# BioinfoMachineLearning/bio-diffusion

Hardware: NVIDIA B200
Metric: molecules/sec (1000-step sample) (higher is better)
Workload: dtype bf16x2 (split hi+lo operands, f32 accumulate; <=1e-4 of the fp32 reference)

## Files before the change

### bio-diffusion_b200/bdiff/_lib.py

```python
from __future__ import annotations

import ctypes as C
import os

_HERE = os.path.dirname(os.path.abspath(__file__))
LIB_PATH = os.path.join(_HERE, "libbdiff_sm100.so")

MODE_PARITY_FP32 = 0
MODE_TENSOR = 1


class BdiffError(RuntimeError):
    pass


class Config(C.Structure):
    _fields_ = [("num_h", C.c_int32), ("num_context", C.c_int32), ("num_layers", C.c_int32),
                ("h_hidden", C.c_int32), ("chi_hidden", C.c_int32), ("e_hidden", C.c_int32),
                ("xi_hidden", C.c_int32), ("mode", C.c_int32)]


PROTOTYPES = {
    "bdiff_abi_version": (C.c_int32, []),
    "bdiff_create": (C.c_int32, [C.POINTER(Config), C.POINTER(C.c_void_p)]),
    "bdiff_destroy": (None, [C.c_void_p]),
    "bdiff_last_error": (C.c_char_p, [C.c_void_p]),
    "bdiff_set_weight": (C.c_int32, [C.c_void_p, C.c_void_p, C.c_char_p, C.c_void_p, C.POINTER(C.c_int64), C.c_int32]),
    "bdiff_weights_missing": (C.c_int32, [C.c_void_p]),
    "bdiff_prepare": (C.c_int32, [C.c_void_p, C.c_void_p]),
    "bdiff_selftest_split": (C.c_int32, [C.c_void_p, C.c_int32, C.c_void_p, C.c_void_p, C.c_void_p]),
    "bdiff_selftest_pair": (C.c_int32, [C.c_void_p, C.c_void_p, C.c_void_p, C.c_void_p]),
    "bdiff_plan_topology": (C.c_int32, [C.c_void_p, C.c_void_p, C.c_int32, C.c_int64, C.c_void_p, C.c_void_p,
                                        C.POINTER(C.c_int64)]),
    "bdiff_edge_index": (C.c_int32, [C.c_void_p, C.c_void_p, C.c_void_p]),
    "bdiff_denoise_forward": (C.c_int32, [C.c_void_p, C.c_void_p, C.c_void_p, C.c_void_p, C.c_void_p, C.c_void_p]),
    "bdiff_profile_forward": (C.c_int32, [C.c_void_p, C.c_void_p, C.c_void_p, C.c_void_p, C.c_void_p, C.c_void_p,
                                          C.POINTER(C.c_float)]),
    "bdiff_debug_tap": (C.c_int32, [C.c_void_p, C.c_void_p, C.c_char_p, C.c_void_p, C.POINTER(C.c_int64),
                                    C.POINTER(C.c_int64)]),
    "bdiff_reverse_step": (C.c_int32, [C.c_void_p, C.c_void_p, C.c_void_p, C.c_void_p, C.c_void_p, C.c_void_p,
                                       C.c_void_p, C.c_void_p]),
    "bdiff_decode_z0": (C.c_int32, [C.c_void_p, C.c_void_p, C.c_void_p, C.c_void_p, C.c_void_p, C.c_void_p,
                                    C.c_void_p, C.c_void_p]),
    "bdiff_center_noise": (C.c_int32, [C.c_void_p, C.c_void_p, C.c_void_p, C.c_void_p, C.c_void_p]),
    "bdiff_check": (C.c_int32, [C.c_void_p, C.c_void_p]),
    "bdiff_check_stability": (C.c_int32, [C.c_void_p] * 4 + [C.c_int32, C.c_int32] + [C.c_void_p] * 3 + [C.c_float] * 3 +
                              [C.c_void_p, C.c_int32, C.c_void_p, C.c_void_p, C.c_void_p]),
    "bdiff_bond_orders": (C.c_int32, [C.c_void_p] * 5 + [C.c_int32, C.c_int32] + [C.c_void_p] * 3 + [C.c_float] * 3 +
                          [C.c_int32, C.c_void_p]),
    "bdiff_collate_count": (C.c_int32, [C.c_void_p, C.c_void_p, C.c_void_p, C.c_int32, C.c_int32, C.c_void_p]),
    "bdiff_collate_packed": (C.c_int32, [C.c_void_p] * 6 + [C.c_int32, C.c_int32, C.c_int32] + [C.c_void_p] * 4),
    "bdiff_prepare_context": (C.c_int32, [C.c_void_p] * 6 + [C.c_int64, C.c_int64, C.c_int32, C.c_void_p]),
    "bdiff_optimizer_chunk": (C.c_int32, []),
    "bdiff_optimizer_step": (C.c_int32, [C.c_void_p, C.c_void_p, C.c_void_p, C.c_void_p, C.c_int32, C.c_void_p, C.c_void_p,
                                         C.c_void_p]),
    "bdiff_param_floats": (C.c_int64, [C.c_void_p]),
    "bdiff_param_layout": (C.c_int32, [C.c_void_p, C.c_char_p, C.POINTER(C.c_int64), C.POINTER(C.c_int64)]),
    "bdiff_train_precision": (C.c_int32, [C.c_void_p, C.c_int32]),
    "bdiff_train_variant": (C.c_int32, [C.c_void_p, C.c_int32]),
    "bdiff_train_timing": (C.c_int32, [C.c_void_p, C.c_void_p, C.c_int32, C.c_char_p, C.c_int64]),
    "bdiff_train_forward": (C.c_int32, [C.c_void_p] * 7),
    "bdiff_train_backward": (C.c_int32, [C.c_void_p] * 4),
    "bdiff_nan_guard_count": (C.c_int32, [C.c_void_p, C.c_void_p, C.POINTER(C.c_int64), C.c_int32]),
    "bdiff_launch_count": (C.c_int64, [C.c_void_p]),
# ... 33 lines not shown
```

### bio-diffusion_b200/csrc/bdiff_api.cu

```cuda
#include <algorithm>
#include <cstdarg>
#include <cstdio>
#include <cstdlib>
#include <cstring>
#include <map>
#include <string>
#include <utility>
#include <vector>

#include "../../include/bdiff.h"
#include "bdiff_handle.h"

using namespace bdiff;

namespace {

thread_local std::string g_create_error;


}

namespace {

void gcp_names(std::map<std::string, bool>& seen, const std::string& p, bool ff, bool vout) {
// ... 139 lines not shown
               o_fbar = take(Np * 12), o_h = take(Np * 256), o_chi = take(Np * 96), o_PI = take(Np * kPStride),
               o_PJ = take(Np * kPStride), o_agg = take(Np * kMsg), o_hp = take(Np * 32),
               o_e = take(Ep * d.Ed), o_xie = take(Ep * d.Xd * 3), o_fr = take(Ep * 9), o_pjt = take(Np * 256),
               o_mid = take(h->cfg.mode == BDIFF_MODE_TENSOR ? (Ep / 128) * kMsg : 0),
               o_flag = take(64);
  cudaError_t e = h->work_buf.ensure(off * sizeof(float));
  if (e != cudaSuccess) return e;
  float* b = static_cast<float*>(h->work_buf.p);
  Work& w = h->work;
  w.x_init = b + o_xi; w.x = b + o_x; w.h_in = b + o_hin; w.chi_in = b + o_chin; w.fbar = b + o_fbar;
  w.h = b + o_h; w.chi = b + o_chi; w.PI = b + o_PI; w.PJ = b + o_PJ; w.agg = b + o_agg; w.hproj = b + o_hp;
  w.e = b + o_e; w.xi = b + o_xie; w.frames = b + o_fr;
  w.PJT = h->cfg.mode == BDIFF_MODE_TENSOR ? b + o_pjt : nullptr;
  w.mid = h->cfg.mode == BDIFF_MODE_TENSOR ? b + o_mid : nullptr;
  w.npad = (int)Np;
  w.nan_flag = reinterpret_cast<int*>(b + o_flag);
  w.dbg = nullptr;
  if (getenv("BDIFF_TIMING")) {
    e = h->dbg_buf.ensure(2 * 256 * 64 * sizeof(long long));
    if (e != cudaSuccess) return e;
    w.dbg = static_cast<long long*>(h->dbg_buf.p);
  }
  e = h->eps_buf.ensure(Np * (3 + d.F) * sizeof(float));
  if (e != cudaSuccess) return e;
  return h->tu_buf.ensure(256);
}

}

extern "C" {

int32_t bdiff_abi_version(void) { return BDIFF_ABI_VERSION; }

const char* bdiff_last_error(const bdiff_handle* h) { return h ? h->err.c_str() : g_create_error.c_str(); }

int32_t bdiff_create(const bdiff_config* cfg, bdiff_handle** out) {
  if (!cfg || !out) { g_create_error = "null argument"; return BDIFF_EINVAL; }
  *out = nullptr;
  if (cfg->h_hidden != 256 || cfg->chi_hidden != 32) { g_create_error = "h_hidden must be 256 and chi_hidden 32"; return BDIFF_EINVAL; }
  if (cfg->e_hidden < 4 || cfg->e_hidden > 64 || cfg->e_hidden % 4) { g_create_error = "e_hidden must be a multiple of 4 in [4,64]"; return BDIFF_EINVAL; }
  if (cfg->xi_hidden < 4 || cfg->xi_hidden > 16 || cfg->xi_hidden % 4) { g_create_error = "xi_hidden must be a multiple of 4 in [4,16]"; return BDIFF_EINVAL; }
  if (cfg->num_h < 1 || cfg->num_context < 0 || cfg->num_h + 1 + cfg->num_context > 28) { g_create_error = "num_h + 1 + num_context must be in [2,28]"; return BDIFF_EINVAL; }
  if (cfg->num_layers < 1 || cfg->num_layers > 64) { g_create_error = "num_layers out of range"; return BDIFF_EINVAL; }
  if (cfg->mode != BDIFF_MODE_PARITY_FP32 && cfg->mode != BDIFF_MODE_TENSOR) { g_create_error = "unknown mode"; return BDIFF_EINVAL; }
  int dev_count = 0;
  if (cudaGetDeviceCount(&dev_count) != cudaSuccess || dev_count == 0) {
    g_create_error = "no CUDA device: libbdiff_sm100 has no CPU fallback";
    return BDIFF_ECUDA;
  }
  cudaDeviceProp prop{};
  int dev = 0;
  cudaGetDevice(&dev);
  cudaGetDeviceProperties(&prop, dev);
  if (prop.major != 10) {
    g_create_error = "libbdiff_sm100 is built for sm_100a (B200) only; found compute capability " +
                     std::to_string(prop.major) + "." + std::to_string(prop.minor);
    return BDIFF_ECUDA;
  }
  bdiff_handle* h = new bdiff_handle();
  h->cfg = *cfg;
  Dims& d = h->d;
  d.F = cfg->num_h; d.C = cfg->num_context; d.Hin = d.F + 1 + d.C; d.Ed = cfg->e_hidden; d.Xd = cfg->xi_hidden;
  d.hid0 = (64 + d.Xd) / 4;
  d.K0 = round_up(d.Ed + d.hid0 + 9, 4);
  d.Ke = round_up(1 + d.Xd + 9, 4);
  d.Kn = round_up(d.Hin + 32 + 9, 4);
// ... 563 lines not shown
```

### bio-diffusion_b200/csrc/bdiff_edge_tc.cuh

```cuda
#pragma once
#include "bdiff_kernels.h"
#include "bdiff_slab.cuh"

namespace bdiff {

constexpr int TMT = 128;
constexpr int TC_SLOT = 2 * 160 * 32;
constexpr int TC_NSLOT = 5;
constexpr int TM_S = 0, TM_U0 = 256, TM_U1 = 288, TM_MV = 320, TM_VD0 = 416;
constexpr int TM_EX = 416, TM_EX_STRIDE = 40;

__host__ __device__ inline int tc_k0_steps(int Ed, int Xd) {
  return (Ed + (64 + Xd) / 4 + 9 + 15) / 16;
}
__host__ __device__ inline size_t tc_edge_stream_bytes(int Ed, int Xd) {
  return (size_t)tc_k0_steps(Ed, Xd) * 2 * 256 * 32 + 3 * ((size_t)16 * 2 * 320 * 32 + 2 * 2 * 256 * 32) + (size_t)16 * 2 * 32 * 32;
}

struct TcBars {
  uint64_t full[TC_NSLOT], empty[TC_NSLOT], pfull[TC_NSLOT], a_ready, d_full, wbar, u_free;
  uint64_t item_full[2], item_empty[2], peer_empty[2], tile_done;
  alignas(16) int item[2][4];
  uint32_t tmem_ptr;
  uint32_t pad_;
};

constexpr int TC_EPI = 256;

struct alignas(16) SmallW {
  float Wd0x[16 * 20];
  float Wf0x[16 * 3];
  float Wu0[20 * 32];
  float Wdk[3][32 * 8];
  float Wfk[3][32 * 3];
  float Wuk[3][8 * 32];
  float bg[4][32];
  float bk[3][256];
  float wa[256];
  float ba[4];
};

struct EdgeTail : TcBars {
  float2 wbuf[2][8][2][32];
  SmallW sw;
  float sAttn[2][TMT];
  int sRow[TMT], sCol[TMT], sB[TMT], sNa[TMT];
  uint32_t winfo[8];
};

template <int HP, bool FIRST, bool LAST>
__device__ __forceinline__ void gate_update(uint32_t tl, int half, int ucol, const float* __restrict__ vdp,
                                            const float* __restrict__ Wu, const float* __restrict__ bgp,
                                            const float* __restrict__ Wdn, const float* __restrict__ Wfn,
// ... 101 lines not shown
```

### bio-diffusion_b200/csrc/bdiff_kernels.h

```cpp
#pragma once
#include <cuda_runtime.h>
#include <stddef.h>

#include "bdiff_common.cuh"

namespace bdiff {

struct Work {
  float* x_init;
  float* x;
  float* h_in;
  float* chi_in;
  float* fbar;
  float* h;
  float* chi;
  float* PI;
  float* PJ;
  float* PJT;
  int npad;
  float* agg;
  float* mid;
  float* hproj;
  float* e;
  float* xi;
  float* frames;
  int* nan_flag;
  long long* dbg;
};

cudaError_t configure_kernels();
size_t edge_smem_bytes();
size_t node_smem_bytes();

void launch_prep(cudaStream_t st, const Plan& p, const Dims& d, const float* xh, const float* t_nodes,
                 const float* coef_table, const int* step_ptr, const float* ctx, const Work& w);
void launch_edge_embed(cudaStream_t st, const Plan& p, const Dims& d, const EmbedW& ew, const Work& w);
void launch_node_embed(cudaStream_t st, const Plan& p, const Dims& d, const EmbedW& ew, const LayerW& l0,
                       const Work& w);
void launch_edge_message(cudaStream_t st, const Plan& p, const Dims& d, const LayerW& lw, const Work& w);
void launch_node_update(cudaStream_t st, const Plan& p, const Dims& d, const LayerW& lw, const LayerW& wn,
                        const EmbedW& ew, const Work& w, int last);
void launch_finalize(cudaStream_t st, const Plan& p, const Dims& d, const Work& w, float* out);
void launch_step(cudaStream_t st, const Plan& p, const Dims& d, int mode, const float* z, const float* eps,
                 const float* noise_x, const float* noise_h, const float* coef_table, const int* step_ptr,
                 float* out);
void launch_edge_index(cudaStream_t st, const Plan& p, long long* out);
void launch_edge_rc(cudaStream_t st, const Plan& p, int4* out, long long n);
struct PackJob {
  float* dst;
  const float* src;
  int dst_ld, src_ld, col0, ncols, kpad, nout;
  int block0;
};
void launch_pack_multi(cudaStream_t st, const PackJob* jobs_dev, int njobs, int total_blocks);

bool tc_supported(int Ed, int Xd);
size_t tc_blob_bytes(int Ed, int Xd);
size_t tc_node_blob_bytes();
void launch_tc_pack(cudaStream_t st, const LayerW& lw, const Dims& d, unsigned char* blob);
void launch_tc_pack_node(cudaStream_t st, const LayerW& lw, const LayerW& wn, const EmbedW& ew, const Dims& d, int last,
                         unsigned char* blob);
struct LayerSched {
  const LayerW* layers;
  const unsigned char* edge_blob;
  size_t edge_blob_stride;
  const unsigned char* node_blob;
  size_t node_blob_stride;
  int L, TE, TN;
  int nitems;
  int* sched;
  int* err;
  const int2* edge_dep;
  const int2* node_dep;
  const int* items;
};
cudaError_t tc_layers_configure();
void launch_layers_tc(cudaStream_t st, const Plan& p, const Dims& d, const EmbedW& ew, const LayerSched& q,
                      const Work& w, int num_sms);
cudaError_t selftest_configure();
cudaError_t selftest_pair_configure();
size_t selftest_pair_img_bytes();
void launch_umma_selftest_pair(cudaStream_t st, const float* A, const float* W, unsigned char* img_scratch, float* C);
size_t selftest_img_bytes();
void launch_umma_selftest_split(cudaStream_t st, const float* A, const float* W, unsigned char* img_scratch, float* C,
                                int variant);

}
```

### bio-diffusion_b200/csrc/bdiff_layers_tc.cu

```cuda
#include "bdiff_node_tc.cuh"

namespace bdiff {

__device__ __forceinline__ int ld_acquire_gpu(const int* p) {
  int v;
  asm volatile("ld.acquire.gpu.global.s32 %0, [%1];" : "=r"(v) : "l"(p) : "memory");
  return v;
}
__device__ __forceinline__ void st_release_gpu(int* p, int v) {
  asm volatile("st.release.gpu.global.s32 [%0], %1;" ::"l"(p), "r"(v) : "memory");
}

union LayersTail {
  TcBars bars;
  EdgeTail edge;
  NodeTail node;
};
constexpr size_t LAYERS_SMEM_BYTES = XE_BLOCKS * (size_t)X_BLOCK + TC_NSLOT * (size_t)TC_SLOT + sizeof(LayersTail) + 1024;
static_assert(LAYERS_SMEM_BYTES <= 232448, "shared memory budget of the layer megakernel");

constexpr int LAYERS_THREADS = 384;
constexpr int LAYERS_REG_COMPUTE = 200, LAYERS_REG_SERVICE = 96;
static_assert(256 * LAYERS_REG_COMPUTE + 128 * LAYERS_REG_SERVICE <= 168 * LAYERS_THREADS, "setmaxnreg pool");

// ... 16 lines not shown
}

template <int ED, int XD>
__global__ void __cluster_dims__(2, 1, 1) __launch_bounds__(LAYERS_THREADS, 1)
    k_layers_tc(Plan p, Dims d, EmbedW ew, LayerSched q, Work w) {
  constexpr int HID0 = (64 + XD) / 4;
  constexpr int H2 = HID0 / 2;
  constexpr int K0RAW = ED + HID0 + 9;
  constexpr int K0S = (K0RAW + 15) / 16;
  static_assert(HID0 % 2 == 0 && H2 * 3 <= 32 && HID0 + 9 <= 32 && ED % 16 == 0, "layout");

  extern __shared__ unsigned char smem_raw[];
  unsigned char* smem = smem_raw + ((1024u - (smem_u32(smem_raw) & 1023u)) & 1023u);
  unsigned char* X = smem;
  unsigned char* ring = smem + XE_BLOCKS * X_BLOCK;
  unsigned char* tail = ring + TC_NSLOT * TC_SLOT;
  TcBars& B = *reinterpret_cast<TcBars*>(tail);
  const int tid = threadIdx.x, warp = tid >> 5, lane = tid & 31;
  const int hid0 = d.hid0;
  const int per_layer = q.TE + q.TN;
  const int total_items = q.nitems;
  int* const flags = q.sched + 2;
  const uint32_t rank = cluster_ctarank();
  const bool leader = rank == 0;

  if (tid == 0) {
    for (int i = 0; i < TC_NSLOT; ++i) { mbar_init(&B.full[i], 1); mbar_init(&B.empty[i], 1); mbar_init(&B.pfull[i], 1); }
    for (int i = 0; i < 2; ++i) {
      mbar_init(&B.item_full[i], 1); mbar_init(&B.item_empty[i], leader ? TC_EPI + 1 : TC_EPI + 2); mbar_init(&B.peer_empty[i], 1);
    }
    mbar_init(&B.tile_done, TC_EPI);
    mbar_init(&B.a_ready, leader ? TC_EPI + 1 : TC_EPI);
    mbar_init(&B.d_full, 1);
    mbar_init(&B.wbar, 1);
    mbar_init(&B.u_free, leader ? TC_EPI + 1 : TC_EPI);
    mbar_fence_init();
  }
  cluster_sync_all();
  if (warp == 8) tmem_alloc2(&B.tmem_ptr, 512);
  tc_fence_before();
  __syncthreads();
  tc_fence_after();
  const uint32_t tmem = B.tmem_ptr;
  const uint32_t a_ready_leader = mapa_u32(&B.a_ready, 0), u_free_leader = mapa_u32(&B.u_free, 0);

  if (warp == 8) {
    asm volatile("setmaxnreg.dec.sync.aligned.u32 %0;\n" ::"n"(LAYERS_REG_SERVICE));
    if (lane == 0) {
      uint32_t ci = 0;
      for (uint32_t k = 0;; ++k) {
        const uint32_t slot = k & 1;
        mbar_wait_backoff(&B.item_empty[slot], ((k >> 1) & 1) ^ 1);
        int type = -1, layer = 0, tile = 0;
        if (leader) {
          mbar_wait_backoff(&B.peer_empty[slot], (k >> 1) & 1);
          const int qi = atomicAdd(q.sched, 1);
          int pair = 0;
          if (qi < total_items) {
            const int it = __ldg(q.items + qi);
            type = (it >> 30) & 1; layer = (it >> 24) & 63; pair = it & 0xffffff;
          }
          B.item[slot][0] = type; B.item[slot][1] = layer; B.item[slot][2] = 2 * pair;
          st_cluster_v4(mapa_u32(&B.item[slot][0], 1), type, layer, 2 * pair + 1, 0);
          mbar_arrive(&B.item_full[slot]);
          mbar_arrive_remote(mapa_u32(&B.item_full[slot], 1));
          tile = 2 * pair;
// ... 3 lines not shown
          type = B.item[slot][0]; layer = B.item[slot][1]; tile = B.item[slot][2];
        }
        (void)tile;
        if (type < 0) break;
        const unsigned char* blob = type == 0 ? q.edge_blob + (size_t)layer * q.edge_blob_stride + rank * (q.edge_blob_stride / 2)
                                              : q.node_blob + (size_t)layer * q.node_blob_stride + rank * (q.node_blob_stride / 2);
        size_t off = 0;
        auto push = [&](uint32_t bytes) {
          const uint32_t s = ci % TC_NSLOT;
          mbar_wait_backoff(&B.empty[s], ((ci / TC_NSLOT) & 1) ^ 1);
          mbar_expect_tx(&B.full[s], bytes);
          bulk_g2s(ring + s * TC_SLOT, blob + off, bytes, &B.full[s]);
          off += bytes;
          ++ci;
        };
        if (type == 0) {
#include "edge_tile_producer.inc"
        } else {
          const int last = layer == q.L - 1;
#include "node_r4_tile_producer.inc"
        }
      }
    }
  } else if (warp == 9 && !leader) {
    asm volatile("setmaxnreg.dec.sync.aligned.u32 %0;\n" ::"n"(LAYERS_REG_SERVICE));
    if (lane < TC_NSLOT) {
      const uint32_t pfull0 = mapa_u32(&B.pfull[0], 0);
      uint32_t ci = 0;
      for (uint32_t k = 0;; ++k) {
        const uint32_t slot = k & 1;
        mbar_wait_cluster(&B.item_full[slot], (k >> 1) & 1);
        const int type = B.item[slot][0], layer = B.item[slot][1], tile = B.item[slot][2];
        if (type < 0) break;
        const uint32_t nch = type == 0 ? K0S + 3 * 18 + 4 : (layer == q.L - 1 ? 73u : 100u);
        for (uint32_t cc = ci + ((lane + TC_NSLOT - ci % TC_NSLOT) % TC_NSLOT); cc < ci + nch; cc += TC_NSLOT) {
          mbar_wait_backoff(&B.full[lane], (cc / TC_NSLOT) & 1);
          mbar_arrive_remote_relaxed(pfull0 + lane * 8);
        }
        ci += nch;
        if (lane == 0) {
          mbar_wait_backoff(&B.tile_done, k & 1);
          __threadfence();
          if (tile < (type == 0 ? q.TE : q.TN))
            st_release_gpu(flags + (size_t)layer * per_layer + (type == 0 ? tile : q.TE + tile), 1);
          mbar_arrive(&B.item_empty[slot]);
        }
      }
    }
  } else if (warp == 9) {
    asm volatile("setmaxnreg.dec.sync.aligned.u32 %0;\n" ::"n"(LAYERS_REG_SERVICE));
    if (lane == 0) {
      TcBars& T = B;
      const uint32_t i256 = umma_idesc_bf16_m256(256), i64 = umma_idesc_bf16_m256(64), i32 = umma_idesc_bf16_m256(32);
      const uint32_t xaddr = smem_u32(X), raddr = smem_u32(ring);
      uint32_t ci = 0, pa = 0, pu = 0;
      long long wcyc = 0, acyc = 0;
      auto wait_a = [&]() {
        if (!leader) return;
        const long long t0 = w.dbg ? clock64() : 0;
        mbar_wait_backoff(&B.a_ready, pa); pa ^= 1;
        tc_fence_after();
        if (w.dbg) acyc += clock64() - t0;
      };
      auto wait_w = [&]() -> uint32_t {
        const uint32_t s = ci % TC_NSLOT, par = (ci / TC_NSLOT) & 1;
        const long long t0 = w.dbg ? clock64() : 0;
        mbar_wait_backoff(&B.full[s], par);
        mbar_wait_backoff(&B.pfull[s], par);
        if (w.dbg) wcyc += clock64() - t0;
        return raddr + s * TC_SLOT;
      };
      auto done_w = [&]() { if (leader) umma_commit_pair(&B.empty[ci % TC_NSLOT]); ++ci; };
      auto commit_d = [&]() { if (leader) umma_commit_pair(&B.d_full); };
      auto mma = [&](uint32_t dcol, uint64_t ad, uint64_t bd, uint32_t idesc, bool acc) { if (leader) umma_bf16_pair(tmem + dcol, ad, bd, idesc, acc); };
      auto ngemm = [&](int NL, uint32_t dcol, bool fresh, int umode) {
        for (int ks = 0; ks < 16; ++ks) {
          const uint32_t a = xaddr + (ks >> 2) * R5_BLOCK + (ks & 3) * 32;
          const uint64_t v0 = umma_desc_sw128(a), v1 = umma_desc_sw128(a + 4096);
          const uint32_t wb0 = wait_w();
          for (int pl = 0; pl < 2; ++pl) {
            const uint32_t wb = wb0 + pl * NL * 32;
            const bool first = ks == 0 && pl == 0;
            const uint64_t bs = umma_desc_k16(wb, NL * 16, 128);
            mma(dcol, v0, bs, i256, fresh ? !first : true);
            mma(dcol, v1, bs, i256, true);
            if (umode) {
              const uint64_t bu = umma_desc_k16(wb + 128 * 16, NL * 16, 128);
              mma(NM_U, v0, bu, i32, umode == 2 ? !first : true);
              mma(NM_U, v1, bu, i32, true);
            }
          }
          done_w();
        }
      };
      auto nextra = [&]() {
        for (int ks = 0; ks < 2; ++ks) {
          const uint32_t a = xaddr + 4 * R5_BLOCK + ks * 32;
          const uint64_t v0 = umma_desc_sw128(a), v1 = umma_desc_sw128(a + 4096);
          const uint32_t wb0 = wait_w();
          for (int pl = 0; pl < 2; ++pl) {
            const uint32_t wb = wb0 + pl * 128 * 32;
            mma(NM_S, v0, umma_desc_k16(wb, 128 * 16, 128), i256, true);
            mma(NM_S, v1, umma_desc_k16(wb, 128 * 16, 128), i256, true);
          }
          done_w();
        }
// ... 15 lines not shown
          long long* o = w.dbg + 256 * 64 + 148 * 64 + (size_t)blockIdx.x * 8 + (k - 2) * 4;
          o[0] = (type << 30) | (layer << 24) | tile; o[1] = clock64() - tstart; o[2] = wcyc; o[3] = acyc;
        }
        mbar_wait_backoff(&B.tile_done, k & 1);
        __threadfence();
        if (tile < (type == 0 ? q.TE : q.TN))
          st_release_gpu(flags + (size_t)layer * per_layer + (type == 0 ? tile : q.TE + tile), 1);
        mbar_arrive(&B.item_empty[slot]);
      }
    }
  } else if (warp == 10) {
    asm volatile("setmaxnreg.dec.sync.aligned.u32 %0;\n" ::"n"(LAYERS_REG_SERVICE));
    if (lane == 0 && !leader) {
      uint32_t pa = 0, pu = 0;
      for (uint32_t k = 0;; ++k) {
        const uint32_t slot = k & 1;
        mbar_wait_cluster(&B.item_full[slot], (k >> 1) & 1);
        const int type = B.item[slot][0], layer = B.item[slot][1];
        if (type < 0) break;
        const bool has_u = type == 1 && layer != q.L - 1;
        const int nph = type == 0 ? 8 : 6;
        for (int ph = 0; ph < nph; ++ph) {
          if (has_u && ph == 4) { mbar_wait_backoff(&B.u_free, pu); pu ^= 1; mbar_arrive_remote_relaxed(u_free_leader); }
          mbar_wait_backoff(&B.a_ready, pa); pa ^= 1;
          mbar_arrive_remote_relaxed(a_ready_leader);
        }
        mbar_arrive(&B.item_empty[slot]);
      }
    }
  } else if (warp >= 11) {
    asm volatile("setmaxnreg.dec.sync.aligned.u32 %0;\n" ::"n"(LAYERS_REG_SERVICE));
  } else {
    asm volatile("setmaxnreg.inc.sync.aligned.u32 %0;\n" ::"n"(LAYERS_REG_COMPUTE));
    uint32_t pd = 0, pw = 0;
    int cur_type = -1, cur_layer = -1;
    int es = 0;
    long long* stamp = nullptr;
    auto PH = [&]() { if (stamp && tid == 0 && es < 32) stamp[es] = clock64(); ++es; };
    auto wait_d = [&]() { PH(); mbar_wait(&B.d_full, pd); pd ^= 1; tc_fence_after(); PH(); };
    auto publish = [&]() { fence_proxy_async(); tc_fence_before(); mbar_arrive(&B.a_ready); PH(); };
    bool stamped[2] = {false, false};
    const uint32_t tl = tmem + ((uint32_t)((warp & 3) * 32) << 16);
    auto sz = [](int n) { return (uint32_t)((n * 4 + 15) & ~15); };
    for (uint32_t k = 0;; ++k) {
      const uint32_t slot = k & 1;
      mbar_wait_cluster(&B.item_full[slot], (k >> 1) & 1);
      const int type = B.item[slot][0], layer = B.item[slot][1], tile = B.item[slot][2];
      if (type < 0) break;
      const bool real = tile < (type == 0 ? q.TE : q.TN);
      if (tid == 0 && w.dbg && k < 16) {
        w.dbg[(size_t)blockIdx.x * 64 + 4 * k] = (type << 30) | (layer << 24) | tile;
        w.dbg[(size_t)blockIdx.x * 64 + 4 * k + 1] = clock64();
      }
      if (type != cur_type || layer != cur_layer) {
        named_bar_sync(3, TC_EPI);
        if (tid == 0) {
          const LayerW lw = q.layers[layer];
          if (type == 0) {
            SmallW& s = reinterpret_cast<EdgeTail*>(tail)->sw;
            mbar_expect_tx(&B.wbar, sz(XD * HID0) + sz(XD * 3) + sz(HID0 * 32) +
                                        3 * (sz(256) + sz(256) + sz(256) + sz(96) + sz(32)) + sz(32) + sz(256) + sz(1));
            auto cp = [&](float* dst, const float* src, int n) { bulk_g2s(dst, src, sz(n), &B.wbar); };
            cp(s.Wd0x, lw.Wd0x, XD * HID0); cp(s.Wf0x, lw.Wf0x, XD * 3); cp(s.Wu0, lw.Wu0, HID0 * 32);
            for (int kk = 0; kk < 3; ++kk) {
              cp(s.Wdk[kk], lw.Wdk[kk], 256); cp(s.Wuk[kk], lw.Wuk[kk], 256); cp(s.bk[kk], lw.bk[kk], 256);
              cp(s.Wfk[kk], lw.Wfk[kk], 96); cp(s.bg[kk + 1], lw.bgk[kk], 32);
            }
            cp(s.bg[0], lw.bg0, 32); cp(s.wa, lw.wa, 256); cp(s.ba, lw.ba, 1);
          } else {
            const int last = layer == q.L - 1;
            const LayerW wn = q.layers[last ? layer : layer + 1];
            SmallWR4& s = reinterpret_cast<NodeTail*>(tail)->sw;
// ... 93 lines not shown
```

### bio-diffusion_b200/csrc/bdiff_tc_pack.cu

```cuda
#include "bdiff_node_tc.cuh"

namespace bdiff {

size_t tc_blob_bytes(int Ed, int Xd) { return tc_edge_stream_bytes(Ed, Xd); }
size_t tc_node_blob_bytes() { return tc_node_stream_bytes(0); }

__global__ void k_pack_edge_slabs(LayerW lw, Dims d, unsigned char* __restrict__ blob, size_t half_bytes) {
  const int K0S = tc_k0_steps(d.Ed, d.Xd);
  const long long rows_g = 16 * 320 + 2 * 256;
  const long long total_rows = (long long)K0S * 256 + 3 * rows_g + 16 * 32;
  const long long idx = (long long)blockIdx.x * blockDim.x + threadIdx.x;
  if (idx >= total_rows * 16) return;
  long long row = idx >> 4;
  const int kk = (int)(idx & 15);
  size_t base = 0;
  int NL, n, k, cta, local;
  float v;
  if (row < (long long)K0S * 256) {
    const int step = (int)(row / 256);
    n = (int)(row % 256); NL = 128; cta = n >> 7; local = n & 127; base = (size_t)step * 2 * 128 * 32; k = step * 16 + kk;
    v = k < d.K0 ? lw.W0e[(size_t)k * 256 + n] : 0.f;
  } else {
    row -= (long long)K0S * 256;
    base = (size_t)K0S * 2 * 128 * 32;
    const size_t bytes_g = (size_t)16 * 2 * 160 * 32 + 2 * 2 * 128 * 32;
    if (row < 3 * rows_g) {
      const int gi = (int)(row / rows_g);
      long long rr = row - gi * rows_g;
      base += gi * bytes_g;
      if (rr < 16 * 320) {
        const int step = (int)(rr / 320);
        n = (int)(rr % 320); NL = 160; base += (size_t)step * 2 * 160 * 32; k = step * 16 + kk;
        const float* wprev = gi == 0 ? lw.Wg0 : lw.Wgk[gi - 1];
        const float* wthis = lw.Wgk[gi];
        const bool odd = ((gi + 1) & 1) != 0;
        if (n < 256) { v = lw.Wk[gi][(size_t)k * 256 + n]; cta = n >> 7; local = n & 127; }
        else if (n < 288) { v = odd ? wprev[(size_t)k * 32 + (n - 256)] : -wthis[(size_t)k * 32 + (n - 256)]; cta = 0; local = 128 + (n - 256); }
        else { v = odd ? -wthis[(size_t)k * 32 + (n - 288)] : wprev[(size_t)k * 32 + (n - 288)]; cta = 1; local = 128 + (n - 288); }
      } else {
        rr -= 16 * 320;
        const int step = (int)(rr / 256);
        n = (int)(rr % 256); NL = 128; cta = n >> 7; local = n & 127;
        base += (size_t)16 * 2 * 160 * 32 + (size_t)step * 2 * 128 * 32; k = 256 + step * 16 + kk;
        v = k < kKM ? lw.Wk[gi][(size_t)k * 256 + n] : 0.f;
      }
    } else {
      row -= 3 * rows_g;
      base += 3 * bytes_g;
      const int step = (int)(row / 32);
      n = (int)(row % 32); NL = 16; cta = n >> 4; local = n & 15; base += (size_t)step * 2 * 16 * 32; k = step * 16 + kk;
      v = lw.Wgk[2][(size_t)k * 32 + n];
    }
  }
  slab_store(blob + (size_t)cta * half_bytes + base, NL, local, kk, v);
}

__global__ void k_pack_node_slabs(LayerW lw, LayerW wn, EmbedW ew, Dims d, int last, unsigned char* __restrict__ blob,
                                  size_t half_bytes) {
  const long long idx = (long long)blockIdx.x * blockDim.x + threadIdx.x;
  long long row = idx >> 4;
  const int kk = (int)(idx & 15);
  size_t base = 0;
  int NL = 0, n = 0, k = 0, cta = 0, local = 0;
  float v = 0.f;
  bool found = false;
  auto seg = [&](int steps, int NN) -> bool {
    if (found) return false;
    const long long rows = (long long)steps * NN;
    const int nl = NN == 256 ? 128 : (NN == 288 ? 144 : 16);
    if (row < rows) {
      const int step = (int)(row / NN);
// ... 43 lines not shown
```

### bio-diffusion_b200/csrc/edge_tile_epilogue.inc

```
      const long long g = (long long)tile * TMT + r;
      constexpr int PV = HID0 * 3 + 9, PF4 = (PV + 3) / 4, PLD = PF4 * 4 + 1;
      constexpr int XF4 = XD * 3 / 4, XLD = XD * 3 + 1;
      static_assert(K0S <= 8 && TMT * XLD * 4 <= 2 * X_BLOCK && TMT * PLD * 4 <= 3 * X_BLOCK, "staging areas");
      float* sFx = reinterpret_cast<float*>(X + 2 * X_BLOCK);
      float* sFp = reinterpret_cast<float*>(X + 6 * X_BLOCK);
      const int4 rc = __ldg(p.edge_rc + g);
      float f[9];
      {
        constexpr int F4_ROW = ED / 4;
        const float4* eb = reinterpret_cast<const float4*>(w.e + (size_t)tile * TMT * ED);
        const float4* xb = reinterpret_cast<const float4*>(w.xi + (size_t)tile * TMT * XD * 3);
        float4 ev[TMT * F4_ROW / TC_EPI], xv[TMT * XF4 / TC_EPI];
#pragma unroll
        for (int i = 0; i < TMT * F4_ROW / TC_EPI; ++i) ev[i] = eb[i * TC_EPI + tid];
#pragma unroll
        for (int i = 0; i < TMT * XF4 / TC_EPI; ++i) xv[i] = xb[i * TC_EPI + tid];
#pragma unroll
        for (int qq = 0; qq < 9; ++qq) f[qq] = w.frames[(size_t)g * 9 + qq];
        if (half == 0) { T.sRow[r] = rc.x; T.sCol[r] = rc.y; T.sB[r] = rc.z; T.sNa[r] = rc.w; }
#pragma unroll
        for (int i = 0; i < TMT * F4_ROW / TC_EPI; ++i) {
          const int idx = i * TC_EPI + tid;
          const int rr = idx / F4_ROW, kk = (idx % F4_ROW) * 4;
          xe_store4(X, rr, kk, ev[i].x, ev[i].y, ev[i].z, ev[i].w);
// ... 98 lines not shown
        auto prefetch = [&](int c) {
          const float* pc = pjt + c * 1024;
#pragma unroll
          for (int i = 0; i < 32; ++i) pj[i] = pc[i * 32];
#pragma unroll
          for (int qq = 0; qq < 8; ++qq) pa[qq] = *reinterpret_cast<const float4*>(pi + half * 128 + c * 32 + qq * 4);
        };
        prefetch(0);
        wait_d();
        for (int c = 0; c < 4; ++c) {
          const int c0 = half * 128 + c * 32;
          float v[32];
          tmem_ld32(tl + TM_S + c0, v);
#pragma unroll
          for (int qq = 0; qq < 8; ++qq) {
            v[qq * 4 + 0] += pa[qq].x + pj[qq * 4 + 0]; v[qq * 4 + 1] += pa[qq].y + pj[qq * 4 + 1];
            v[qq * 4 + 2] += pa[qq].z + pj[qq * 4 + 2]; v[qq * 4 + 3] += pa[qq].w + pj[qq * 4 + 3];
          }
          if (c < 3) prefetch(c + 1);
#pragma unroll
          for (int qq = 0; qq < 16; ++qq) {
            const float2 p0 = silu_acc2(make_float2(v[2 * qq], v[2 * qq + 1]));
            v[2 * qq] = p0.x; v[2 * qq + 1] = p0.y;
          }
#pragma unroll
          for (int qq = 0; qq < 4; ++qq) xe_store8(X, r, c0 + qq * 8, v + qq * 8);
        }
      }
      publish();

      float vd[24], vdf[9];
      float2 adot2 = make_float2(0.f, 0.f);
      for (int k = 1; k <= 3; ++k) {
        wait_d();
        float part[33], other[33];
        if (k == 1) {
          float vd0[HID0 * 3];
          {
            float t0[64];
            float* t1 = t0 + 32;
            tmem_ld64(tl + TM_VD0, t0);
#pragma unroll
            for (int i = 0; i < H2 * 3; ++i) { vd0[i] = t0[i]; vd0[H2 * 3 + i] = t1[i]; }
          }
          tc_fence_before();
          named_bar_sync(3, TC_EPI);
          tc_fence_after();
          gate_update<HID0, true, false>(tl, half, TM_U0, vd0, sw.Wu0, sw.bg[0], sw.Wdk[0], sw.Wfk[0], part);
        } else {
          gate_update<8, false, false>(tl, half, ((k - 1) & 1) ? TM_U1 : TM_U0, vd, sw.Wuk[k - 2], sw.bg[k - 1],
                                       sw.Wdk[k - 1], sw.Wfk[k - 1], part);
        }
        pair_exchange33(tl, half, part, other);
#pragma unroll
        for (int i = 0; i < 24; ++i) vd[i] = half == 0 ? part[i] + other[i] : other[i] + part[i];
#pragma unroll
        for (int i = 0; i < 9; ++i) vdf[i] = half == 0 ? part[24 + i] + other[24 + i] : other[24 + i] + part[24 + i];
        {
          float a[16];
          if (half == 0) {
#pragma unroll
            for (int h = 0; h < 8; ++h) a[h] = safe_norm3(vd[h * 3], vd[h * 3 + 1], vd[h * 3 + 2]);
#pragma unroll
            for (int i = 0; i < 8; ++i) {
              const int ch = i / 3, ax = i - ch * 3;
              a[8 + i] = f[ax * 3] * vdf[ch * 3] + f[ax * 3 + 1] * vdf[ch * 3 + 1] + f[ax * 3 + 2] * vdf[ch * 3 + 2];
            }
// ... 166 lines not shown
```

### bio-diffusion_b200/csrc/edge_tile_mma.inc

```
        {
          const uint32_t xe = xaddr + XE_EXTRA * X_BLOCK;
          wait_a();
          for (int ks = 0; ks < K0S; ++ks) {
            const uint64_t ah = umma_desc_sw128(xaddr + (ks >> 2) * X_BLOCK + (ks & 3) * 32);
            const uint64_t al = umma_desc_sw128(xaddr + (XE_LO + (ks >> 2)) * X_BLOCK + (ks & 3) * 32);
            const uint32_t bh = wait_w(), bl = bh + 128 * 32;
            mma(TM_S, ah, umma_desc_k16(bh, 128 * 16, 128), i256, ks > 0);
            mma(TM_S, al, umma_desc_k16(bh, 128 * 16, 128), i256, true);
            mma(TM_S, ah, umma_desc_k16(bl, 128 * 16, 128), i256, true);
            done_w();
          }
          commit_d();
          for (int k = 1; k <= 3; ++k) {
            wait_a();
            for (int ks = 0; ks < 16; ++ks) {
              const uint64_t ah = umma_desc_sw128(xaddr + (ks >> 2) * X_BLOCK + (ks & 3) * 32);
              const uint64_t al = umma_desc_sw128(xaddr + (XE_LO + (ks >> 2)) * X_BLOCK + (ks & 3) * 32);
              const uint32_t bh = wait_w(), bl = bh + 160 * 32;
              mma(TM_S, ah, umma_desc_k16(bh, 160 * 16, 128), i256, ks > 0);
              mma(TM_U0, ah, umma_desc_k16(bh + 128 * 16, 160 * 16, 128), i64, k == 1 ? ks > 0 : true);
              mma(TM_S, al, umma_desc_k16(bh, 160 * 16, 128), i256, true);
              mma(TM_U0, al, umma_desc_k16(bh + 128 * 16, 160 * 16, 128), i64, true);
              mma(TM_S, ah, umma_desc_k16(bl, 160 * 16, 128), i256, true);
              mma(TM_U0, ah, umma_desc_k16(bl + 128 * 16, 160 * 16, 128), i64, true);
              done_w();
            }
            commit_d();
            wait_a();
            for (int ks = 0; ks < 2; ++ks) {
              const uint64_t ah = umma_desc_sw128(xe + ks * 32), al = umma_desc_sw128(xe + 64 + ks * 32);
              const uint32_t bh = wait_w(), bl = bh + 128 * 32;
              mma(TM_S, ah, umma_desc_k16(bh, 128 * 16, 128), i256, true);
              mma(TM_S, al, umma_desc_k16(bh, 128 * 16, 128), i256, true);
              mma(TM_S, ah, umma_desc_k16(bl, 128 * 16, 128), i256, true);
              done_w();
            }
            commit_d();
          }
          wait_a();
          for (int c = 0; c < 4; ++c) {
            const uint32_t wb = wait_w();
            for (int s4 = 0; s4 < 4; ++s4) {
              const int ks = c * 4 + s4;
              const uint64_t ah = umma_desc_sw128(xaddr + (ks >> 2) * X_BLOCK + (ks & 3) * 32);
              const uint64_t al = umma_desc_sw128(xaddr + (XE_LO + (ks >> 2)) * X_BLOCK + (ks & 3) * 32);
              const uint32_t bh = wb + s4 * 1024, bl = bh + 512;
              mma(TM_U1, ah, umma_desc_k16(bh, 16 * 16, 128), i32, true);
              mma(TM_U1, al, umma_desc_k16(bh, 16 * 16, 128), i32, true);
              mma(TM_U1, ah, umma_desc_k16(bl, 16 * 16, 128), i32, true);
            }
            done_w();
          }
          commit_d();
        }
```

### bio-diffusion_b200/csrc/edge_tile_producer.inc

```
        for (int ks = 0; ks < K0S; ++ks) push(2 * 128 * 32);
        for (int k = 0; k < 3; ++k) {
          for (int ks = 0; ks < 16; ++ks) push(2 * 160 * 32);
          for (int ks = 0; ks < 2; ++ks) push(2 * 128 * 32);
        }
        for (int c = 0; c < 4; ++c) push(4 * 2 * 16 * 32);
```

### include/bdiff.h

```cpp
#ifndef BDIFF_H_
#define BDIFF_H_

#include <stdint.h>

#ifdef __cplusplus
extern "C" {
#endif

#define BDIFF_OK 0
#define BDIFF_EINVAL (-1)
#define BDIFF_ECUDA (-2)
#define BDIFF_ESTATE (-3)
#define BDIFF_ENOMEM (-4)

#define BDIFF_ABI_VERSION 1

#if defined(__GNUC__)
#define BDIFF_API __attribute__((visibility("default")))
#else
#define BDIFF_API
#endif

#define BDIFF_MODE_PARITY_FP32 0
#define BDIFF_MODE_TENSOR 1

typedef struct bdiff_handle bdiff_handle;

typedef struct bdiff_config {
  int32_t num_h;
  int32_t num_context;
  int32_t num_layers;
  int32_t h_hidden;
  int32_t chi_hidden;
  int32_t e_hidden;
  int32_t xi_hidden;
  int32_t mode;
} bdiff_config;

BDIFF_API int32_t bdiff_abi_version(void);

BDIFF_API int32_t bdiff_create(const bdiff_config* cfg, bdiff_handle** out);
BDIFF_API void bdiff_destroy(bdiff_handle* h);
BDIFF_API const char* bdiff_last_error(const bdiff_handle* h);

BDIFF_API int32_t bdiff_set_weight(bdiff_handle* h, void* stream, const char* name, const float* data,
                         const int64_t* shape, int32_t ndim);
BDIFF_API int32_t bdiff_weights_missing(const bdiff_handle* h);

BDIFF_API int32_t bdiff_prepare(bdiff_handle* h, void* stream);

BDIFF_API int32_t bdiff_selftest_split(void* stream, int32_t variant, const float* A, const float* W, float* C);

BDIFF_API int32_t bdiff_selftest_pair(void* stream, const float* A, const float* W, float* C);

BDIFF_API int32_t bdiff_plan_topology(bdiff_handle* h, void* stream, int32_t num_mols, int64_t num_nodes,
                            const int64_t* batch_index, const uint8_t* mask, int64_t* num_edges_host);

BDIFF_API int32_t bdiff_edge_index(bdiff_handle* h, void* stream, int64_t* edge_index);

BDIFF_API int32_t bdiff_denoise_forward(bdiff_handle* h, void* stream, const float* xh, const float* t,
                              const float* context, float* net_out);

BDIFF_API int32_t bdiff_profile_forward(bdiff_handle* h, void* stream, const float* xh, const float* t,
                                        const float* context, float* net_out, float* ms_host);

BDIFF_API int32_t bdiff_debug_tap(bdiff_handle* h, void* stream, const char* which, float* dst, int64_t* rows,
                                  int64_t* cols);

BDIFF_API int32_t bdiff_reverse_step(bdiff_handle* h, void* stream, float* z, const float* context,
                                     const float* noise_x, const float* noise_h, const float* coef_table,
                                     const int32_t* step_index);

BDIFF_API int32_t bdiff_decode_z0(bdiff_handle* h, void* stream, const float* z0, const float* context,
                                  const float* noise_x, const float* noise_h, const float* coef, float* xh);

BDIFF_API int32_t bdiff_center_noise(bdiff_handle* h, void* stream, const float* noise_x, const float* noise_h,
                                     float* z);

BDIFF_API int32_t bdiff_check(bdiff_handle* h, void* stream);

#define BDIFF_OPT_MAX_QUEUE 120
#define BDIFF_OPT_STATE_WORDS (8 + BDIFF_OPT_MAX_QUEUE)
typedef struct bdiff_opt_tensor {
  float* param;
  const float* grad;
  float* exp_avg;
// ... 55 lines not shown
```

Before: 60.86.

## Split edge GCP weight stream so U-gate GEMM completes early on own barrier

Repacks the edge-tile weight stream so the 32-column U/gate weights for each GCP are streamed as separate chunks ahead of the 256-column scalar weights. The MMA warp computes the U accumulator first and signals a new u_full barrier, letting the epilogue start its vector work while the scalar GEMM is still running, instead of waiting on a single combined commit. This changes the packed blob layout, the chunk count and the producer sequence, and adds a host-visible layout query. It risks more pipeline chunks and smaller per-MMA N for the U part.

```diff
diff --git a/bio-diffusion_b200/bdiff/_lib.py b/bio-diffusion_b200/bdiff/_lib.py
--- a/bio-diffusion_b200/bdiff/_lib.py
+++ b/bio-diffusion_b200/bdiff/_lib.py
@@ -30,6 +30,7 @@
     "bdiff_prepare": (C.c_int32, [C.c_void_p, C.c_void_p]),
     "bdiff_selftest_split": (C.c_int32, [C.c_void_p, C.c_int32, C.c_void_p, C.c_void_p, C.c_void_p]),
     "bdiff_selftest_pair": (C.c_int32, [C.c_void_p, C.c_void_p, C.c_void_p, C.c_void_p]),
+    "bdiff_tc_edge_stream_layout": (C.c_int32, [C.c_int32, C.c_int32, C.POINTER(C.c_int64)]),
     "bdiff_plan_topology": (C.c_int32, [C.c_void_p, C.c_void_p, C.c_int32, C.c_int64, C.c_void_p, C.c_void_p,
                                         C.POINTER(C.c_int64)]),
     "bdiff_edge_index": (C.c_int32, [C.c_void_p, C.c_void_p, C.c_void_p]),
diff --git a/bio-diffusion_b200/csrc/bdiff_api.cu b/bio-diffusion_b200/csrc/bdiff_api.cu
--- a/bio-diffusion_b200/csrc/bdiff_api.cu
+++ b/bio-diffusion_b200/csrc/bdiff_api.cu
@@ -195,6 +195,12 @@
 
 int32_t bdiff_abi_version(void) { return BDIFF_ABI_VERSION; }
 
+int32_t bdiff_tc_edge_stream_layout(int32_t e_hidden, int32_t xi_hidden, int64_t* out) {
+  if (!out || !tc_supported(e_hidden, xi_hidden)) return BDIFF_EINVAL;
+  tc_edge_stream_layout(e_hidden, xi_hidden, out);
+  return 0;
+}
+
 const char* bdiff_last_error(const bdiff_handle* h) { return h ? h->err.c_str() : g_create_error.c_str(); }
 
 int32_t bdiff_create(const bdiff_config* cfg, bdiff_handle** out) {
diff --git a/bio-diffusion_b200/csrc/bdiff_edge_tc.cuh b/bio-diffusion_b200/csrc/bdiff_edge_tc.cuh
--- a/bio-diffusion_b200/csrc/bdiff_edge_tc.cuh
+++ b/bio-diffusion_b200/csrc/bdiff_edge_tc.cuh
@@ -10,15 +10,31 @@
 constexpr int TM_S = 0, TM_U0 = 256, TM_U1 = 288, TM_MV = 320, TM_VD0 = 416;
 constexpr int TM_EX = 416, TM_EX_STRIDE = 40;
 
-__host__ __device__ inline int tc_k0_steps(int Ed, int Xd) {
+__host__ __device__ constexpr int tc_k0_steps(int Ed, int Xd) {
   return (Ed + (64 + Xd) / 4 + 9 + 15) / 16;
 }
-__host__ __device__ inline size_t tc_edge_stream_bytes(int Ed, int Xd) {
+__host__ __device__ constexpr size_t tc_edge_stream_bytes(int Ed, int Xd) {
   return (size_t)tc_k0_steps(Ed, Xd) * 2 * 256 * 32 + 3 * ((size_t)16 * 2 * 320 * 32 + 2 * 2 * 256 * 32) + (size_t)16 * 2 * 32 * 32;
 }
 
+constexpr uint32_t TC_EC_S = 2 * 128 * 32, TC_EC_U = 4 * 2 * 32 * 32, TC_EC_G4 = 4 * 2 * 16 * 32;
+constexpr int TC_EC_PER_GCP = 4 + 16 + 2;
+__host__ __device__ constexpr int tc_edge_tile_chunks(int k0s) { return k0s + 3 * TC_EC_PER_GCP + 4; }
+__host__ __device__ constexpr uint32_t tc_edge_chunk_bytes(int k0s, int c) {
+  return c < k0s ? TC_EC_S : c < k0s + 3 * TC_EC_PER_GCP ? ((c - k0s) % TC_EC_PER_GCP < 4 ? TC_EC_U : TC_EC_S) : TC_EC_G4;
+}
+__host__ __device__ constexpr size_t tc_edge_chunks_total_bytes(int k0s) {
+  size_t b = 0;
+  for (int c = 0; c < tc_edge_tile_chunks(k0s); ++c) b += tc_edge_chunk_bytes(k0s, c);
+  return 2 * b;
+}
+static_assert(tc_edge_chunks_total_bytes(tc_k0_steps(64, 16)) == tc_edge_stream_bytes(64, 16) &&
+              tc_edge_chunks_total_bytes(tc_k0_steps(16, 8)) == tc_edge_stream_bytes(16, 8),
+              "edge chunk table and packed stream size disagree");
+static_assert(TC_EC_S <= TC_SLOT && TC_EC_U <= TC_SLOT && TC_EC_G4 <= TC_SLOT, "an edge chunk fits one ring slot");
+
 struct TcBars {
-  uint64_t full[TC_NSLOT], empty[TC_NSLOT], pfull[TC_NSLOT], a_ready, d_full, wbar, u_free;
+  uint64_t full[TC_NSLOT], empty[TC_NSLOT], pfull[TC_NSLOT], a_ready, d_full, wbar, u_free, u_full;
   uint64_t item_full[2], item_empty[2], peer_empty[2], tile_done;
   alignas(16) int item[2][4];
   uint32_t tmem_ptr;
diff --git a/bio-diffusion_b200/csrc/bdiff_kernels.h b/bio-diffusion_b200/csrc/bdiff_kernels.h
--- a/bio-diffusion_b200/csrc/bdiff_kernels.h
+++ b/bio-diffusion_b200/csrc/bdiff_kernels.h
@@ -56,6 +56,7 @@
 
 bool tc_supported(int Ed, int Xd);
 size_t tc_blob_bytes(int Ed, int Xd);
+void tc_edge_stream_layout(int Ed, int Xd, int64_t* out);
 size_t tc_node_blob_bytes();
 void launch_tc_pack(cudaStream_t st, const LayerW& lw, const Dims& d, unsigned char* blob);
 void launch_tc_pack_node(cudaStream_t st, const LayerW& lw, const LayerW& wn, const EmbedW& ew, const Dims& d, int last,
diff --git a/bio-diffusion_b200/csrc/bdiff_layers_tc.cu b/bio-diffusion_b200/csrc/bdiff_layers_tc.cu
--- a/bio-diffusion_b200/csrc/bdiff_layers_tc.cu
+++ b/bio-diffusion_b200/csrc/bdiff_layers_tc.cu
@@ -72,6 +72,7 @@
     mbar_init(&B.tile_done, TC_EPI);
     mbar_init(&B.a_ready, leader ? TC_EPI + 1 : TC_EPI);
     mbar_init(&B.d_full, 1);
+    mbar_init(&B.u_full, 1);
     mbar_init(&B.wbar, 1);
     mbar_init(&B.u_free, leader ? TC_EPI + 1 : TC_EPI);
     mbar_fence_init();
@@ -141,7 +142,7 @@
         mbar_wait_cluster(&B.item_full[slot], (k >> 1) & 1);
         const int type = B.item[slot][0], layer = B.item[slot][1], tile = B.item[slot][2];
         if (type < 0) break;
-        const uint32_t nch = type == 0 ? K0S + 3 * 18 + 4 : (layer == q.L - 1 ? 73u : 100u);
+        const uint32_t nch = type == 0 ? (uint32_t)tc_edge_tile_chunks(K0S) : (layer == q.L - 1 ? 73u : 100u);
         for (uint32_t cc = ci + ((lane + TC_NSLOT - ci % TC_NSLOT) % TC_NSLOT); cc < ci + nch; cc += TC_NSLOT) {
           mbar_wait_backoff(&B.full[lane], (cc / TC_NSLOT) & 1);
           mbar_arrive_remote_relaxed(pfull0 + lane * 8);
@@ -181,6 +182,7 @@
       };
       auto done_w = [&]() { if (leader) umma_commit_pair(&B.empty[ci % TC_NSLOT]); ++ci; };
       auto commit_d = [&]() { if (leader) umma_commit_pair(&B.d_full); };
+      auto commit_u = [&]() { if (leader) umma_commit_pair(&B.u_full); };
       auto mma = [&](uint32_t dcol, uint64_t ad, uint64_t bd, uint32_t idesc, bool acc) { if (leader) umma_bf16_pair(tmem + dcol, ad, bd, idesc, acc); };
       auto ngemm = [&](int NL, uint32_t dcol, bool fresh, int umode) {
         for (int ks = 0; ks < 16; ++ks) {
@@ -262,12 +264,13 @@
     asm volatile("setmaxnreg.dec.sync.aligned.u32 %0;\n" ::"n"(LAYERS_REG_SERVICE));
   } else {
     asm volatile("setmaxnreg.inc.sync.aligned.u32 %0;\n" ::"n"(LAYERS_REG_COMPUTE));
-    uint32_t pd = 0, pw = 0;
+    uint32_t pd = 0, pg = 0, pw = 0;
     int cur_type = -1, cur_layer = -1;
     int es = 0;
     long long* stamp = nullptr;
     auto PH = [&]() { if (stamp && tid == 0 && es < 32) stamp[es] = clock64(); ++es; };
     auto wait_d = [&]() { PH(); mbar_wait(&B.d_full, pd); pd ^= 1; tc_fence_after(); PH(); };
+    auto wait_u = [&]() { PH(); mbar_wait(&B.u_full, pg); pg ^= 1; tc_fence_after(); PH(); };
     auto publish = [&]() { fence_proxy_async(); tc_fence_before(); mbar_arrive(&B.a_ready); PH(); };
     bool stamped[2] = {false, false};
     const uint32_t tl = tmem + ((uint32_t)((warp & 3) * 32) << 16);
diff --git a/bio-diffusion_b200/csrc/bdiff_tc_pack.cu b/bio-diffusion_b200/csrc/bdiff_tc_pack.cu
--- a/bio-diffusion_b200/csrc/bdiff_tc_pack.cu
+++ b/bio-diffusion_b200/csrc/bdiff_tc_pack.cu
@@ -4,6 +4,12 @@
 
 size_t tc_blob_bytes(int Ed, int Xd) { return tc_edge_stream_bytes(Ed, Xd); }
 size_t tc_node_blob_bytes() { return tc_node_stream_bytes(0); }
+void tc_edge_stream_layout(int Ed, int Xd, int64_t* out) {
+  const int k0s = tc_k0_steps(Ed, Xd);
+  out[0] = (int64_t)tc_edge_stream_bytes(Ed, Xd);
+  out[1] = tc_edge_tile_chunks(k0s);
+  out[2] = (int64_t)tc_edge_chunks_total_bytes(k0s);
+}
 
 __global__ void k_pack_edge_slabs(LayerW lw, Dims d, unsigned char* __restrict__ blob, size_t half_bytes) {
   const int K0S = tc_k0_steps(d.Ed, d.Xd);
@@ -30,13 +36,18 @@
       base += gi * bytes_g;
       if (rr < 16 * 320) {
         const int step = (int)(rr / 320);
-        n = (int)(rr % 320); NL = 160; base += (size_t)step * 2 * 160 * 32; k = step * 16 + kk;
+        n = (int)(rr % 320); k = step * 16 + kk;
         const float* wprev = gi == 0 ? lw.Wg0 : lw.Wgk[gi - 1];
         const float* wthis = lw.Wgk[gi];
         const bool odd = ((gi + 1) & 1) != 0;
-        if (n < 256) { v = lw.Wk[gi][(size_t)k * 256 + n]; cta = n >> 7; local = n & 127; }
-        else if (n < 288) { v = odd ? wprev[(size_t)k * 32 + (n - 256)] : -wthis[(size_t)k * 32 + (n - 256)]; cta = 0; local = 128 + (n - 256); }
-        else { v = odd ? -wthis[(size_t)k * 32 + (n - 288)] : wprev[(size_t)k * 32 + (n - 288)]; cta = 1; local = 128 + (n - 288); }
+        if (n < 256) {
+          v = lw.Wk[gi][(size_t)k * 256 + n]; cta = n >> 7; local = n & 127;
+          NL = 128; base += (size_t)16 * 2 * 32 * 32 + (size_t)step * 2 * 128 * 32;
+        } else {
+          if (n < 288) { v = odd ? wprev[(size_t)k * 32 + (n - 256)] : -wthis[(size_t)k * 32 + (n - 256)]; cta = 0; local = n - 256; }
+          else { v = odd ? -wthis[(size_t)k * 32 + (n - 288)] : wprev[(size_t)k * 32 + (n - 288)]; cta = 1; local = n - 288; }
+          NL = 32; base += (size_t)step * 2 * 32 * 32;
+        }
       } else {
         rr -= 16 * 320;
         const int step = (int)(rr / 256);
diff --git a/bio-diffusion_b200/csrc/edge_tile_epilogue.inc b/bio-diffusion_b200/csrc/edge_tile_epilogue.inc
--- a/bio-diffusion_b200/csrc/edge_tile_epilogue.inc
+++ b/bio-diffusion_b200/csrc/edge_tile_epilogue.inc
@@ -154,7 +154,7 @@
       float vd[24], vdf[9];
       float2 adot2 = make_float2(0.f, 0.f);
       for (int k = 1; k <= 3; ++k) {
-        wait_d();
+        wait_u();
         float part[33], other[33];
         if (k == 1) {
           float vd0[HID0 * 3];
diff --git a/bio-diffusion_b200/csrc/edge_tile_mma.inc b/bio-diffusion_b200/csrc/edge_tile_mma.inc
--- a/bio-diffusion_b200/csrc/edge_tile_mma.inc
+++ b/bio-diffusion_b200/csrc/edge_tile_mma.inc
@@ -13,19 +13,29 @@
           commit_d();
           for (int k = 1; k <= 3; ++k) {
             wait_a();
+            for (int c = 0; c < 4; ++c) {
+              const uint32_t wb = wait_w();
+              for (int s4 = 0; s4 < 4; ++s4) {
+                const int ks = c * 4 + s4;
+                const uint64_t ah = umma_desc_sw128(xaddr + (ks >> 2) * X_BLOCK + (ks & 3) * 32);
+                const uint64_t al = umma_desc_sw128(xaddr + (XE_LO + (ks >> 2)) * X_BLOCK + (ks & 3) * 32);
+                const uint32_t bh = wb + s4 * 2048, bl = bh + 1024;
+                mma(TM_U0, ah, umma_desc_k16(bh, 32 * 16, 128), i64, k == 1 ? ks > 0 : true);
+                mma(TM_U0, al, umma_desc_k16(bh, 32 * 16, 128), i64, true);
+                mma(TM_U0, ah, umma_desc_k16(bl, 32 * 16, 128), i64, true);
+              }
+              done_w();
+            }
+            commit_u();
             for (int ks = 0; ks < 16; ++ks) {
               const uint64_t ah = umma_desc_sw128(xaddr + (ks >> 2) * X_BLOCK + (ks & 3) * 32);
               const uint64_t al = umma_desc_sw128(xaddr + (XE_LO + (ks >> 2)) * X_BLOCK + (ks & 3) * 32);
-              const uint32_t bh = wait_w(), bl = bh + 160 * 32;
-              mma(TM_S, ah, umma_desc_k16(bh, 160 * 16, 128), i256, ks > 0);
-              mma(TM_U0, ah, umma_desc_k16(bh + 128 * 16, 160 * 16, 128), i64, k == 1 ? ks > 0 : true);
-              mma(TM_S, al, umma_desc_k16(bh, 160 * 16, 128), i256, true);
-              mma(TM_U0, al, umma_desc_k16(bh + 128 * 16, 160 * 16, 128), i64, true);
-              mma(TM_S, ah, umma_desc_k16(bl, 160 * 16, 128), i256, true);
-              mma(TM_U0, ah, umma_desc_k16(bl + 128 * 16, 160 * 16, 128), i64, true);
+              const uint32_t bh = wait_w(), bl = bh + 128 * 32;
+              mma(TM_S, ah, umma_desc_k16(bh, 128 * 16, 128), i256, ks > 0);
+              mma(TM_S, al, umma_desc_k16(bh, 128 * 16, 128), i256, true);
+              mma(TM_S, ah, umma_desc_k16(bl, 128 * 16, 128), i256, true);
               done_w();
             }
-            commit_d();
             wait_a();
             for (int ks = 0; ks < 2; ++ks) {
               const uint64_t ah = umma_desc_sw128(xe + ks * 32), al = umma_desc_sw128(xe + 64 + ks * 32);
diff --git a/bio-diffusion_b200/csrc/edge_tile_producer.inc b/bio-diffusion_b200/csrc/edge_tile_producer.inc
--- a/bio-diffusion_b200/csrc/edge_tile_producer.inc
+++ b/bio-diffusion_b200/csrc/edge_tile_producer.inc
@@ -1,6 +1 @@
-        for (int ks = 0; ks < K0S; ++ks) push(2 * 128 * 32);
-        for (int k = 0; k < 3; ++k) {
-          for (int ks = 0; ks < 16; ++ks) push(2 * 160 * 32);
-          for (int ks = 0; ks < 2; ++ks) push(2 * 128 * 32);
-        }
-        for (int c = 0; c < 4; ++c) push(4 * 2 * 16 * 32);
+        for (int c = 0; c < tc_edge_tile_chunks(K0S); ++c) push(tc_edge_chunk_bytes(K0S, c));
diff --git a/include/bdiff.h b/include/bdiff.h
--- a/include/bdiff.h
+++ b/include/bdiff.h
@@ -52,6 +52,8 @@
 BDIFF_API int32_t bdiff_selftest_split(void* stream, int32_t variant, const float* A, const float* W, float* C);
 
 BDIFF_API int32_t bdiff_selftest_pair(void* stream, const float* A, const float* W, float* C);
+
+BDIFF_API int32_t bdiff_tc_edge_stream_layout(int32_t e_hidden, int32_t xi_hidden, int64_t* out);
 
 BDIFF_API int32_t bdiff_plan_topology(bdiff_handle* h, void* stream, int32_t num_mols, int64_t num_nodes,
                             const int64_t* batch_index, const uint8_t* mask, int64_t* num_edges_host);
```

New measurement: 66.18, median of 6. 1.09x the previous value.
